# HarborC/PL-SLAM

Measured on NVIDIA H100. Metric: frames/sec (extract+match+pose-LM) 640x480, higher is better.
Workload: dtype u8/i32 front-end, f32 descriptors, f64 LM

## Files before the change

include/plslam_b200.h:

```cpp
#ifndef PLSLAM_B200_H
#define PLSLAM_B200_H
#include <stddef.h>
#include <stdint.h>
#ifdef __cplusplus
extern "C" {
#endif

#define PL_OK 0
#define PL_ERR_ARG (-1)
#define PL_ERR_CUDA (-2)
#define PL_ERR_CAPACITY (-3)

const char* pl_last_error(void);
int pl_version(void);
unsigned long long pl_launch_count(void);

typedef struct PLKeyPoint {
  float x, y, size, angle, response;
  int32_t octave, class_id;
} PLKeyPoint;

typedef struct PLOrbConfig {
  int width, height;
  int nfeatures;
  float scale_factor;
  int nlevels;
  int ini_th_fast;
  int min_th_fast;
  int max_batch;
  int cell_slot_cap;
} PLOrbConfig;

typedef struct PLOrb PLOrb;

int pl_orb_create(const PLOrbConfig* cfg, PLOrb** out);
void pl_orb_destroy(PLOrb* h);
int pl_orb_capacity(const PLOrb* h);
int pl_orb_tables(const PLOrb* h, float* scale, float* inv_scale, float* sigma2, float* inv_sigma2,
                  int* features_per_level, int* level_w, int* level_h);
int pl_orb_extract(PLOrb* h, const uint8_t* img, int stride, PLKeyPoint* kps, uint8_t* desc, int* n);
int pl_orb_extract_batch(PLOrb* h, const uint8_t* imgs, int stride, size_t frame_stride, int B,
                         PLKeyPoint* kps, uint8_t* desc, int* n);
int pl_orb_extract_batch_dev(PLOrb* h, const uint8_t* imgs, int stride, size_t frame_stride, int B,
                             PLKeyPoint* kps, uint8_t* desc, int* n, void* stream);
int pl_orb_get_level(PLOrb* h, int frame, int level, uint8_t* out, int with_border);
int pl_orb_check_overflow(PLOrb* h);
int pl_orb_debug_candidates(PLOrb* h, int frame, int level, PLKeyPoint* out, int cap);


int pl_descriptor_distance_batch(const uint8_t* a, const uint8_t* b, int n, int* out);

int pl_frame_assign_grid(const PLKeyPoint* keys_un, int n, const float* bounds, int* cell_start, int* cell_items);
int pl_frame_assign_grid_dev(const PLKeyPoint* keys_un, const int* n, int cap, int B, const float* bounds,
                             int* cell_start , int* cell_items , void* stream);

int pl_orb_search_for_initialization(const PLKeyPoint* keys1, const uint8_t* desc1, int n1, const PLKeyPoint* keys2,
                                     const uint8_t* desc2, int n2, const float* bounds, float* prev_matched,
                                     int* matches12, int window_size, float nnratio, int check_orientation);
int pl_orb_search_for_initialization_dev(const PLKeyPoint* keys1, const uint8_t* desc1, const int* n1,
                                         const PLKeyPoint* keys2, const uint8_t* desc2, const int* n2, int cap, int B,
                                         const float* bounds, float* prev_matched, int* matches12, int* nmatches,
                                         int window_size, float nnratio, int check_orientation, int* scratch,
                                         void* stream);

int pl_orb_search_by_projection_last(const PLKeyPoint* keys_cur, const uint8_t* desc_cur, int n_cur,
                                     const float* bounds, const float* Tcw, const float* K,
                                     const float* scale_factors, int nlevels, int n_last, const uint8_t* last_valid,
                                     const float* last_pos, const uint8_t* last_desc, const int* last_octave,
                                     const float* last_angle, float th, int check_orientation,
                                     const uint8_t* cur_preassigned, int* cur_match);

int pl_orb_search_by_projection_points(const PLKeyPoint* keys, const uint8_t* desc, int n, const float* bounds,
                                       const float* scale_factors, int nlevels, int n_mp, const uint8_t* in_view,
                                       const float* proj, const int* level, const float* view_cos,
                                       const uint8_t* mp_desc, float th, float nnratio, const uint8_t* preassigned,
                                       int* match);

int pl_match_bf_knn2(const uint8_t* d1, int n1, const uint8_t* d2, int n2, int* idx, int* dist);
int pl_lsd_frame_bf_match(const uint8_t* d1, int n1, const uint8_t* d2, int n2, float th, float nnratio, int* matches);
int pl_lsd_search_double(const uint8_t* d1, int n1, const uint8_t* d2, int n2, float nnratio, int* matches);
int pl_lsd_search_double_dev(const uint8_t* d1, const int* n1, const uint8_t* d2, const int* n2, int cap1, int cap2,
                             int B, float th, float nnratio, int mutual, int* matches , int* nmatches,
                             void* stream);

int pl_pose_optimization(int mode, const float* Tcw_in, const float* K, int n_points, const float* pt_obs,
                         const float* pt_inv_sigma2, const float* pt_Xw, int n_lines, const double* line_func,
                         const double* line_Xw, float* Tcw_out, uint8_t* pt_outlier, uint8_t* line_outlier,
                         int* iterations );
size_t pl_pose_optimization_scratch_doubles(int B, int cap_points, int cap_lines);
int pl_pose_optimization_dev(int mode, int B, const float* Tcw_in, const float* K, const int* n_points,
                             int cap_points, const float* pt_obs, const float* pt_inv_sigma2, const float* pt_Xw,
                             const int* n_lines, int cap_lines, const double* line_func, const double* line_Xw,
                             float* Tcw_out, uint8_t* pt_outlier, uint8_t* line_outlier, int* inliers,
                             int* iterations, double* scratch, void* stream);

typedef struct PLLineConfig {
  int width, height;
  int nfeatures;
  double min_line_length;
  int max_batch;
  int segment_cap;
  int lsd_used_in_global;
} PLLineConfig;
typedef struct PLLine PLLine;
int pl_line_create(const PLLineConfig* cfg, PLLine** out);
void pl_line_destroy(PLLine* h);
int pl_line_capacity(const PLLine* h);
int pl_line_extract(PLLine* h, const uint8_t* img, int stride, const uint8_t* mask, void* keylines, uint8_t* desc,
                    double* linefunc, int* n);
int pl_line_extract_batch(PLLine* h, const uint8_t* imgs, int stride, size_t frame_stride, int B, const uint8_t* mask,
                          void* keylines, uint8_t* desc, double* linefunc, int* n);
int pl_line_extract_batch_dev(PLLine* h, const uint8_t* imgs, int stride, size_t frame_stride, int B,
                              const uint8_t* mask, void* keylines, uint8_t* desc, double* linefunc, int* n, void* stream);
int pl_line_check_overflow(PLLine* h);
int pl_line_debug_segments(PLLine* h, int frame, float* out, int cap);
int pl_line_debug_scaled(PLLine* h, int frame, uint8_t* out, int* sw, int* sh);
int pl_line_debug_sobel(PLLine* h, int frame, short* dx, short* dy);
int pl_line_debug_order(PLLine* h, int frame, unsigned* out, int cap);
int pl_line_debug_seed_path(PLLine* h);
int pl_line_debug_fill_order(PLLine* h, int byte);

typedef struct PLFrontendConfig {
  int width, height, max_batch;
  int orb_nfeatures; float orb_scale_factor; int orb_nlevels, orb_ini_th, orb_min_th;
  int line_nfeatures; double line_min_length;
  int lm_cap_points, lm_cap_lines;
} PLFrontendConfig;
typedef struct PLFrontend PLFrontend;
int pl_frontend_create(const PLFrontendConfig* cfg, PLFrontend** out);
void pl_frontend_destroy(PLFrontend* h);
// ... 239 lines not shown
```

pl-slam_b200/binding.py:

```python
import ctypes as C
import os
import numpy as np

_HERE = os.path.dirname(os.path.abspath(__file__))
LIB_PATH = os.environ.get("PLSLAM_B200_LIB") or os.path.join(_HERE, "libplslam_b200.so")

KP_DTYPE = np.dtype([("x", "<f4"), ("y", "<f4"), ("size", "<f4"), ("angle", "<f4"),
                     ("response", "<f4"), ("octave", "<i4"), ("class_id", "<i4")])


class PLError(RuntimeError):
    pass


class PLOrbConfig(C.Structure):
    _fields_ = [("width", C.c_int), ("height", C.c_int), ("nfeatures", C.c_int), ("scale_factor", C.c_float),
                ("nlevels", C.c_int), ("ini_th_fast", C.c_int), ("min_th_fast", C.c_int), ("max_batch", C.c_int),
                ("cell_slot_cap", C.c_int)]


_lib = None
vp = C.c_void_p


def lib():
    global _lib
    if _lib is None:
        if not os.path.exists(LIB_PATH):
            raise PLError(f"{LIB_PATH} is missing: run __graft_entry__.build() (no CPU fallback exists)")
        L = C.CDLL(LIB_PATH)
        L.pl_last_error.restype = C.c_char_p
        L.pl_launch_count.restype = C.c_ulonglong
        L.pl_orb_create.argtypes = [C.POINTER(PLOrbConfig), C.POINTER(vp)]
        L.pl_orb_destroy.argtypes = [vp]
        L.pl_orb_capacity.argtypes = [vp]
        L.pl_orb_tables.argtypes = [vp] * 8
        L.pl_orb_extract.argtypes = [vp, vp, C.c_int, vp, vp, vp]
        L.pl_orb_extract_batch.argtypes = [vp, vp, C.c_int, C.c_size_t, C.c_int, vp, vp, vp]
        L.pl_orb_extract_batch_dev.argtypes = [vp, vp, C.c_int, C.c_size_t, C.c_int, vp, vp, vp, vp]
        L.pl_orb_get_level.argtypes = [vp, C.c_int, C.c_int, vp, C.c_int]
        L.pl_orb_debug_candidates.argtypes = [vp, C.c_int, C.c_int, vp, C.c_int]
        _lib = L
    return _lib


def check(rc):
    if rc < 0:
        raise PLError(f"plslam_b200 error {rc}: {lib().pl_last_error().decode()}")
    return rc


def _p(a):
    return a.ctypes.data_as(vp) if a is not None else None


def launch_count():
    return int(lib().pl_launch_count())


class ORBextractor:

    def __init__(self, nfeatures, scaleFactor, nlevels, iniThFAST, minThFAST, width=640, height=480, max_batch=1,
                 cell_slot_cap=0):
        self.cfg = PLOrbConfig(width, height, nfeatures, scaleFactor, nlevels, iniThFAST, minThFAST, max_batch,
                               cell_slot_cap)
        self._h = vp()
        check(lib().pl_orb_create(C.byref(self.cfg), C.byref(self._h)))
        self.capacity = check(lib().pl_orb_capacity(self._h))
        n = nlevels
        self._scale, self._inv, self._s2, self._is2 = (np.zeros(n, np.float32) for _ in range(4))
        self.mnFeaturesPerLevel = np.zeros(n, np.int32)
        self.level_w, self.level_h = np.zeros(n, np.int32), np.zeros(n, np.int32)
        check(lib().pl_orb_tables(self._h, _p(self._scale), _p(self._inv), _p(self._s2), _p(self._is2),
                                  _p(self.mnFeaturesPerLevel), _p(self.level_w), _p(self.level_h)))

    def __del__(self):
        if getattr(self, "_h", None) and self._h.value:
            lib().pl_orb_destroy(self._h)
            self._h = vp()

    def GetLevels(self): return self.cfg.nlevels
    def GetScaleFactor(self): return self.cfg.scale_factor
    def GetScaleFactors(self): return self._scale
    def GetInverseScaleFactors(self): return self._inv
    def GetScaleSigmaSquares(self): return self._s2
    def GetInverseScaleSigmaSquares(self): return self._is2

    def __call__(self, image, mask=None):
        image = np.ascontiguousarray(image, np.uint8)
        if image.size == 0:
            return np.zeros(0, KP_DTYPE), np.zeros((0, 32), np.uint8)
        assert image.shape == (self.cfg.height, self.cfg.width)
        kps = np.zeros(self.capacity, KP_DTYPE)
        desc = np.zeros((self.capacity, 32), np.uint8)
        n = C.c_int(0)
        check(lib().pl_orb_extract(self._h, _p(image), image.strides[0], _p(kps), _p(desc), C.byref(n)))
        return kps[:n.value].copy(), desc[:n.value].copy()

    def extract_batch(self, images):
        images = np.ascontiguousarray(images, np.uint8)
        B = images.shape[0]
        kps = np.zeros((B, self.capacity), KP_DTYPE)
        desc = np.zeros((B, self.capacity, 32), np.uint8)
        n = np.zeros(B, np.int32)
        check(lib().pl_orb_extract_batch(self._h, _p(images), images.strides[1], images.strides[0], B, _p(kps),
                                         _p(desc), _p(n)))
        return kps, desc, n

    def extract_batch_dev(self, img_ptr, stride, frame_stride, B, kps_ptr, desc_ptr, n_ptr, stream=None):
        check(lib().pl_orb_extract_batch_dev(self._h, img_ptr, stride, frame_stride, B, kps_ptr, desc_ptr, n_ptr,
                                             stream))

    def mvImagePyramid(self, level, frame=0, with_border=False):
        w, h = int(self.level_w[level]), int(self.level_h[level])
        if with_border:
            w, h = w + 38, h + 38
        out = np.zeros((h, w), np.uint8)
        check(lib().pl_orb_get_level(self._h, frame, level, _p(out), int(with_border)))
        return out

    def debug_candidates(self, level, frame=0):
        n = check(lib().pl_orb_debug_candidates(self._h, frame, level, None, 0))
        out = np.zeros(max(n, 1), KP_DTYPE)
        check(lib().pl_orb_debug_candidates(self._h, frame, level, _p(out), n))
        return out[:n]


def _u8(a):
    return np.ascontiguousarray(a, np.uint8)


def _f32(a):
    return np.ascontiguousarray(a, np.float32)


def _i32(a):
    return np.ascontiguousarray(a, np.int32)


def frame_assign_grid(keys_un, bounds):
    keys = np.ascontiguousarray(keys_un); b = _f32(bounds)
    start = np.zeros(64 * 48 + 1, np.int32); items = np.zeros(max(len(keys), 1), np.int32)
    check(lib().pl_frame_assign_grid(_p(keys), len(keys), _p(b), _p(start), _p(items)))
    return start, items[:start[-1]]


class ORBmatcher:
    TH_HIGH, TH_LOW, HISTO_LENGTH = 100, 50, 30

    def __init__(self, nnratio=0.6, checkOri=True):
        self.mfNNratio, self.mbCheckOrientation = float(nnratio), bool(checkOri)

    @staticmethod
    def DescriptorDistance(a, b):
        a, b = _u8(a).reshape(-1, 32), _u8(b).reshape(-1, 32)
        out = np.zeros(len(a), np.int32)
        check(lib().pl_descriptor_distance_batch(_p(a), _p(b), len(a), _p(out)))
        return out if len(out) > 1 else int(out[0])

    def SearchForInitialization(self, keys1, desc1, keys2, desc2, bounds, vbPrevMatched, windowSize=10):
        k1, k2 = np.ascontiguousarray(keys1), np.ascontiguousarray(keys2)
        d1, d2 = _u8(desc1), _u8(desc2)
        pm = _f32(vbPrevMatched).copy(); b = _f32(bounds)
        m = np.zeros(max(len(k1), 1), np.int32)
        f = lib().pl_orb_search_for_initialization
        f.argtypes = [vp, vp, C.c_int, vp, vp, C.c_int, vp, vp, vp, C.c_int, C.c_float, C.c_int]
        nm = check(f(_p(k1), _p(d1), len(k1), _p(k2), _p(d2), len(k2), _p(b), _p(pm), _p(m), int(windowSize),
                     self.mfNNratio, int(self.mbCheckOrientation)))
        return nm, m[:len(k1)], pm

    def SearchByProjectionLast(self, keys_cur, desc_cur, bounds, Tcw, K, scale_factors, last_valid, last_pos,
                               last_desc, last_octave, last_angle, th, preassigned=None):
        kc, dc = np.ascontiguousarray(keys_cur), _u8(desc_cur)
        arr = [_f32(bounds), _f32(Tcw), _f32(K), _f32(scale_factors), _u8(last_valid), _f32(last_pos), _u8(last_desc),
               _i32(last_octave), _f32(last_angle)]
        pre = None if preassigned is None else _u8(preassigned)
        m = np.zeros(max(len(kc), 1), np.int32)
        f = lib().pl_orb_search_by_projection_last
        f.argtypes = [vp, vp, C.c_int, vp, vp, vp, vp, C.c_int, C.c_int, vp, vp, vp, vp, vp, C.c_float, C.c_int, vp, vp]
        nm = check(f(_p(kc), _p(dc), len(kc), _p(arr[0]), _p(arr[1]), _p(arr[2]), _p(arr[3]), len(arr[3]), len(arr[4]),
                     _p(arr[4]), _p(arr[5]), _p(arr[6]), _p(arr[7]), _p(arr[8]), float(th),
                     int(self.mbCheckOrientation), _p(pre), _p(m)))
        return nm, m[:len(kc)]

    def SearchByProjectionPoints(self, keys, desc, bounds, scale_factors, in_view, proj, level, view_cos, mp_desc, th=3,
                                 preassigned=None):
        k, d = np.ascontiguousarray(keys), _u8(desc)
        arr = [_f32(bounds), _f32(scale_factors), _u8(in_view), _f32(proj), _i32(level), _f32(view_cos), _u8(mp_desc)]
        pre = None if preassigned is None else _u8(preassigned)
        m = np.zeros(max(len(k), 1), np.int32)
        f = lib().pl_orb_search_by_projection_points
        f.argtypes = [vp, vp, C.c_int, vp, vp, C.c_int, C.c_int, vp, vp, vp, vp, vp, C.c_float, C.c_float, vp, vp]
        nm = check(f(_p(k), _p(d), len(k), _p(arr[0]), _p(arr[1]), len(arr[1]), len(arr[2]), _p(arr[2]), _p(arr[3]),
                     _p(arr[4]), _p(arr[5]), _p(arr[6]), float(th), self.mfNNratio, _p(pre), _p(m)))
        return nm, m[:len(k)]


class LSDmatcher:
    TH_HIGH, TH_LOW = 80, 50

    def __init__(self, nnratio=0.7, checkOri=True):
        self.mfNNratio, self.mbCheckOrientation = float(nnratio), bool(checkOri)

    DescriptorDistance = ORBmatcher.DescriptorDistance

    @staticmethod
    def knnMatch(d1, d2):
        d1, d2 = _u8(d1), _u8(d2)
# ... 1110 lines not shown
```

pl-slam_b200/csrc/orb.cu:

```cuda

#include "common.cuh"
#include "tma.cuh"
#include "libm_glibc.cuh"
#include <math.h>
#include <vector>
#include <algorithm>
#include <string.h>

namespace pl {

constexpr int kMaxLevels = 12;
constexpr int kEdge = 19;
constexpr int kHalfPatch = 15;
constexpr int kMaxWin = 72;

__device__ char4 g_pattern[256];
__constant__ int c_umax[16];
static const int8_t h_pattern[256 * 4] = {
#include "../data/orb_pattern_31.inc"
};

struct LevelInfo {
  int w, h, pitch;
  long long off;
// ... 46 lines not shown
    int sx = tx.x, sx1 = min(sx + 1, sw - 1);
    int r0 = S0[sx] * tx.y + S0[sx1] * tx.z;
    int r1 = S1[sx] * tx.y + S1[sx1] * tx.z;
    o[k] = (uint8_t)((((b0 * (r0 >> 4)) >> 16) + ((b1 * (r1 >> 4)) >> 16) + 2) >> 2);
  }
  if (x4 + 3 < dw) {
    *reinterpret_cast<uchar4*>(D + x4) = make_uchar4(o[0], o[1], o[2], o[3]);
  } else {
    for (int k = 0; x4 + k < dw; k++) D[x4 + k] = o[k];
  }
}

__host__ __device__ __forceinline__ int fast_score_px(const uint8_t* p, int pitch, int minTh) {
  int v = p[0];
  int d0 = v - p[3 * pitch], d8 = v - p[-3 * pitch];
  if (abs(d0) <= minTh && abs(d8) <= minTh) return 0;
  int d4 = v - p[3], d12 = v - p[-3];
  if (abs(d4) <= minTh && abs(d12) <= minTh) return 0;
  int d[16];
  d[0] = d0; d[1] = v - p[3 * pitch + 1]; d[2] = v - p[2 * pitch + 2]; d[3] = v - p[pitch + 3];
  d[4] = d4; d[5] = v - p[-pitch + 3]; d[6] = v - p[-2 * pitch + 2]; d[7] = v - p[-3 * pitch + 1];
  d[8] = d8; d[9] = v - p[-3 * pitch - 1]; d[10] = v - p[-2 * pitch - 2]; d[11] = v - p[-pitch - 3];
  d[12] = d12; d[13] = v - p[pitch - 3]; d[14] = v - p[2 * pitch - 2]; d[15] = v - p[3 * pitch - 1];
  int e[16];
#pragma unroll
  for (int k = 0; k < 16; k++) e[k] = -d[k];
  int a2[16], b2[16], a4[16], b4[16];
#pragma unroll
  for (int k = 0; k < 16; k++) { a2[k] = min(d[k], d[(k + 1) & 15]); b2[k] = min(e[k], e[(k + 1) & 15]); }
#pragma unroll
  for (int k = 0; k < 16; k++) { a4[k] = min(a2[k], a2[(k + 2) & 15]); b4[k] = min(b2[k], b2[(k + 2) & 15]); }
  int bestA = -256, bestB = -256;
#pragma unroll
  for (int k = 0; k < 16; k++) {
    int a9 = min(min(a4[k], a4[(k + 4) & 15]), d[(k + 8) & 15]);
    int b9 = min(min(b4[k], b4[(k + 4) & 15]), e[(k + 8) & 15]);
    bestA = max(bestA, a9);
    bestB = max(bestB, b9);
  }
  int best = bestA > bestB ? bestA : bestB;
  int s = best - 1;
  return s >= minTh ? s : 0;
}

__device__ __forceinline__ unsigned fast_score_pair(const uint8_t* p, int pitch, int minTh) {
  auto pair = [&](int off) { return (unsigned)p[off] | ((unsigned)p[off + 1] << 16); };
  const unsigned negv = __vneg2(pair(0));
  unsigned d[16];
  d[0] = pair(3 * pitch); d[1] = pair(3 * pitch + 1); d[2] = pair(2 * pitch + 2); d[3] = pair(pitch + 3);
  d[4] = pair(3); d[5] = pair(-pitch + 3); d[6] = pair(-2 * pitch + 2); d[7] = pair(-3 * pitch + 1);
  d[8] = pair(-3 * pitch); d[9] = pair(-3 * pitch - 1); d[10] = pair(-2 * pitch - 2); d[11] = pair(-pitch - 3);
  d[12] = pair(-3); d[13] = pair(pitch - 3); d[14] = pair(2 * pitch - 2); d[15] = pair(3 * pitch - 1);
#pragma unroll
  for (int k = 0; k < 16; k++) d[k] = __vadd2(d[k], negv);
  unsigned m3[16], M3[16];
#pragma unroll
  for (int k = 0; k < 16; k++) {
    m3[k] = __vimin3_s16x2(d[k], d[(k + 1) & 15], d[(k + 2) & 15]);
    M3[k] = __vimax3_s16x2(d[k], d[(k + 1) & 15], d[(k + 2) & 15]);
  }
  unsigned best = 0x80008000u, worst = 0x7fff7fffu;
#pragma unroll
  for (int k = 0; k < 16; k += 2) {
    const unsigned a0 = __vimin3_s16x2(m3[k], m3[(k + 3) & 15], m3[(k + 6) & 15]);
    const unsigned a1 = __vimin3_s16x2(m3[k + 1], m3[(k + 4) & 15], m3[(k + 7) & 15]);
    const unsigned b0 = __vimax3_s16x2(M3[k], M3[(k + 3) & 15], M3[(k + 6) & 15]);
    const unsigned b1 = __vimax3_s16x2(M3[k + 1], M3[(k + 4) & 15], M3[(k + 7) & 15]);
    best = __vimax3_s16x2(best, a0, a1);
    worst = __vimin3_s16x2(worst, b0, b1);
  }
  unsigned out = 0;
#pragma unroll
  for (int hv = 0; hv < 2; hv++) {
    const int bb = (int)(short)(best >> (16 * hv)), ww = (int)(short)(worst >> (16 * hv));
    const int nw = 0 - ww;
    const int sc = (bb > nw ? bb : nw) - 1;
    out |= (unsigned)(sc >= minTh ? sc : 0) << (16 * hv);
  }
  return out;
}

constexpr int kFastPitchMax = 96;

__global__ void __launch_bounds__(128) k_fast_cells(OrbParams P, unsigned bulk, const CellInfo* __restrict__ cells,
                                                    const uint8_t* __restrict__ img0, int stride0, long long frame0,
                                                    const uint8_t* __restrict__ pyr, uint32_t* __restrict__ slots,
                                                    int* __restrict__ counts, int* __restrict__ overflow) {
  __shared__ __align__(128) uint8_t win_s[kMaxWin * kFastPitchMax];
  __shared__ __align__(16) uint8_t sc[kMaxWin * kFastPitchMax];
  __shared__ __align__(8) unsigned long long mbar;
  __shared__ int wsum[4];
  const int cell = blockIdx.x, frame = blockIdx.y, tid = threadIdx.x;
  CellInfo c = cells[cell];
  const LevelInfo& L = P.lv[c.level];
  const int w = c.x1 - c.x0, h = c.y1 - c.y0;
  const uint8_t* img;
  int pitch;
  if (c.level == 0) { img = img0 + (long long)frame * frame0; pitch = stride0; }
  else { img = pyr + (long long)frame * P.pyr_frame + L.off; pitch = L.pitch; }
  constexpr int WP = kFastPitchMax;
  const uint8_t* win = win_s;
  if ((bulk >> c.level) & 1u) {
    const int x0a = c.x0 & ~15, rowbytes = ((c.x1 + 15) & ~15) - x0a;
    win = win_s + (c.x0 - x0a);
    if (tid == 0) {
      tma::mbar_init(&mbar, 1);
      tma::fence_mbar_init();
      tma::mbar_expect_tx(&mbar, (unsigned)(rowbytes * h));
    }
    __syncthreads();
    if (tid < h) tma::bulk_load(win_s + tid * WP, img + (long long)(c.y0 + tid) * pitch + x0a, (unsigned)rowbytes, &mbar);
    for (int i = tid; i < (WP * h + 3) / 4; i += 128) reinterpret_cast<unsigned*>(sc)[i] = 0u;
    tma::mbar_wait(&mbar, 0);
  } else {
    const float inv_w = 1.0f / (float)w;
    for (int i = tid; i < w * h; i += 128) {
      const int y = __float2int_rz(__fmul_rn((float)i + 0.5f, inv_w)), x = i - y * w;
      win_s[y * WP + x] = img[(long long)(c.y0 + y) * pitch + c.x0 + x];
    }
    for (int i = tid; i < (WP * h + 3) / 4; i += 128) reinterpret_cast<unsigned*>(sc)[i] = 0u;
  }
  __syncthreads();
  const int dw = w - 6, dh = h - 6;
  const int npx = (dw > 0 && dh > 0) ? dw * dh : 0;
  const float inv_dw = dw > 0 ? 1.0f / (float)dw : 0.f;
  {
    const int pw = (dw + 1) >> 1, npair = (dw > 0 && dh > 0) ? pw * dh : 0;
    const float inv_pw = pw > 0 ? 1.0f / (float)pw : 0.f;
    for (int j = tid; j < npair; j += 128) {
      const int y = __float2int_rz(__fmul_rn((float)j + 0.5f, inv_pw)), x = 2 * (j - y * pw);
      const unsigned s2 = fast_score_pair(&win[(y + 3) * WP + x + 3], WP, P.minTh);
      sc[(y + 3) * WP + x + 3] = (uint8_t)(s2 & 0xffu);
      if (x + 1 < dw) sc[(y + 3) * WP + x + 4] = (uint8_t)(s2 >> 16);
    }
  }
  __syncthreads();
  int n20 = 0;
  uint8_t fl[ (kMaxWin * kMaxWin + 127) / 128 ];
  int nfl = 0;
  const int ppt = (npx + 127) / 128;
  const int beg = tid * ppt, end = min(beg + ppt, npx);
  for (int i = beg; i < end; i++) {
    int y = __float2int_rz(__fmul_rn((float)i + 0.5f, inv_dw)), x = i - y * dw;
    const uint8_t* s = &sc[(y + 3) * WP + x + 3];
    int v = s[0];
    uint8_t f = 0;
    if (v > 0 && v > s[-1] && v > s[1] && v > s[-WP - 1] && v > s[-WP] && v > s[-WP + 1] && v > s[WP - 1] &&
        v > s[WP] && v > s[WP + 1]) {
      f = (v >= P.iniTh) ? 2 : 1;
      n20 += (f == 2);
    }
    fl[nfl++] = f;
  }
  const int tot20 = __syncthreads_count(n20 > 0);
  const uint8_t need = tot20 > 0 ? 2 : 1;
  int mycount = 0;
  for (int k = 0; k < nfl; k++) mycount += (fl[k] >= need);
  int lane = tid & 31, wid = tid >> 5;
  int incl = mycount;
#pragma unroll
  for (int o = 1; o < 32; o <<= 1) { int t = __shfl_up_sync(0xffffffffu, incl, o); if (lane >= o) incl += t; }
  if (lane == 31) wsum[wid] = incl;
  __syncthreads();
  int base = 0, total = 0;
#pragma unroll
  for (int k = 0; k < 4; k++) { if (k < wid) base += wsum[k]; total += wsum[k]; }
  int pos = base + incl - mycount;
  uint32_t* out = slots + ((long long)frame * P.ncells + cell) * P.slotcap;
  for (int k = 0; k < nfl; k++) {
    if (fl[k] >= need) {
      int i = beg + k;
      int y = __float2int_rz(__fmul_rn((float)i + 0.5f, inv_dw)), x = i - y * dw;
      if (pos < P.slotcap)
        out[pos] = (uint32_t)(x + 3 + c.sx) | ((uint32_t)(y + 3 + c.sy) << 12) | ((uint32_t)sc[(y + 3) * WP + x + 3] << 24);
      pos++;
    }
  }
  if (tid == 0) {
    counts[(long long)frame * P.ncells + cell] = min(total, P.slotcap);
    if (total > P.slotcap) atomicExch(overflow, 1);
  }
}

struct QNode {
  short x0, y0, x1, y1;
  int beg, cnt;
  short prev, next;
  unsigned seq;
  unsigned char buf, noMore;
  short pad;
};
constexpr short QNIL = -1;

struct QState {
  QNode* nodes;
  short* freel;
  int nfree;
  short head, tail;
  int size;
  unsigned seq;
};

__device__ __forceinline__ short q_alloc(QState& s) { return s.freel[--s.nfree]; }
__device__ __forceinline__ void q_free(QState& s, short id, int lane) {
  if (lane == 0) s.freel[s.nfree] = id;
  s.nfree++;
}
__device__ __forceinline__ void q_push_front(QState& s, short id, int lane) {
  if (lane == 0) {
    s.nodes[id].prev = QNIL;
    s.nodes[id].next = s.head;
    if (s.head != QNIL) s.nodes[s.head].prev = id;
  }
  if (s.head == QNIL) s.tail = id;
  s.head = id;
  s.size++;
}
__device__ __forceinline__ void q_push_back(QState& s, short id, int lane) {
  if (lane == 0) {
    s.nodes[id].next = QNIL;
    s.nodes[id].prev = s.tail;
    if (s.tail != QNIL) s.nodes[s.tail].next = id;
  }
  if (s.tail == QNIL) s.head = id;
  s.tail = id;
  s.size++;
}
__device__ __forceinline__ void q_erase(QState& s, short id, int lane) {
  short p = s.nodes[id].prev, n = s.nodes[id].next;
  __syncwarp();
  if (lane == 0) {
    if (p != QNIL) s.nodes[p].next = n;
    if (n != QNIL) s.nodes[n].prev = p;
  }
  if (p == QNIL) s.head = n;
  if (n == QNIL) s.tail = p;
  s.size--;
  q_free(s, id, lane);
  __syncwarp();
}

__device__ void q_divide(QState& s, short id, uint32_t* kA, uint32_t* kB, short* vs, int& nv, int& nToExpand,
                         int lane) {
  QNode nd = s.nodes[id];
  const int halfX = (nd.x1 - nd.x0 + 1) >> 1;
  const int halfY = (nd.y1 - nd.y0 + 1) >> 1;
  const int sxp = nd.x0 + halfX, syp = nd.y0 + halfY;
  const uint32_t* src = (nd.buf ? kB : kA) + nd.beg;
  uint32_t* dst = (nd.buf ? kA : kB) + nd.beg;
  int c[4] = {0, 0, 0, 0};
  for (int i = lane; i < nd.cnt; i += 32) {
    uint32_t k = src[i];
    int kx = k & 0xfff, ky = (k >> 12) & 0xfff;
    int q = (kx < sxp) ? ((ky < syp) ? 0 : 2) : ((ky < syp) ? 1 : 3);
    c[q]++;
  }
#pragma unroll
  for (int q = 0; q < 4; q++) c[q] = warp_sum(c[q]);
  int b[4];
// ... 274 lines not shown
  if (level < 0) return;
  const LevelInfo& L = P.lv[level];
  const uint8_t* img;
  int pitch;
  if (level == 0) { img = img0 + (long long)frame * frame0; pitch = stride0; }
  else { img = pyr + (long long)frame * P.pyr_frame + L.off; pitch = L.pitch; }
  const uint32_t key = sel[((long long)frame * P.nlevels + level) * P.selcap + rank];
  const int px = (int)(key & 0xfff) + (kEdge - 3), py = (int)((key >> 12) & 0xfff) + (kEdge - 3);
  const int resp = (int)(key >> 24);
  int m10, m01 = 0;
  {
    const int u = lane - kHalfPatch;
    const uint8_t* c0 = img + (long long)py * pitch + px + u;
    int colsum = 0;
#pragma unroll
    for (int v = -kHalfPatch; v <= kHalfPatch; v++) {
      if (lane <= 2 * kHalfPatch && abs(u) <= c_umax[abs(v)]) {
        const int p = c0[v * pitch];
        colsum += p; m01 += v * p;
      }
    }
    m10 = warp_sum(u * colsum);
    m01 = warp_sum(m01);
  }
  const float angle = fast_atan2_deg((float)m01, (float)m10);
  const float factorPI = (float)(3.1415926535897932384626433832795 / 180.f);
  const float ang = __fmul_rn(angle, factorPI);
  float a = 0.f, b = 0.f;
  if (lane == 0) glibc::sincosf_(ang, &b, &a);
  a = __shfl_sync(0xffffffffu, a, 0); b = __shfl_sync(0xffffffffu, b, 0);
  const int bp = L.bpitch;
  const uint8_t* ctr = blur + (long long)frame * P.blur_frame + L.boff + (long long)py * bp + px;
  int val = 0;
#pragma unroll
  for (int k = 0; k < 8; k++) {
    const char4 pt = __ldg(&g_pattern[lane * 8 + k]);
    float x0 = (float)pt.x, y0 = (float)pt.y, x1 = (float)pt.z, y1 = (float)pt.w;
    int r0 = __float2int_rn(__fadd_rn(__fmul_rn(x0, b), __fmul_rn(y0, a)));
    int c0 = __float2int_rn(__fsub_rn(__fmul_rn(x0, a), __fmul_rn(y0, b)));
    int r1 = __float2int_rn(__fadd_rn(__fmul_rn(x1, b), __fmul_rn(y1, a)));
    int c1 = __float2int_rn(__fsub_rn(__fmul_rn(x1, a), __fmul_rn(y1, b)));
    int t0 = ctr[r0 * bp + c0], t1 = ctr[r1 * bp + c1];
    val |= (t0 < t1) << k;
  }
  desc[((long long)frame * P.cap + idx) * 32 + lane] = (uint8_t)val;
  if (lane == 0) {
    PLKeyPoint kp;
    kp.x = (float)px; kp.y = (float)py;
    if (level != 0) { kp.x = __fmul_rn(kp.x, L.scale); kp.y = __fmul_rn(kp.y, L.scale); }
    kp.size = L.size; kp.angle = angle; kp.response = (float)resp; kp.octave = level; kp.class_id = -1;
    kps[(long long)frame * P.cap + idx] = kp;
  }
}

}

using namespace pl;

struct PLOrb {
  PLOrbConfig cfg;
  OrbParams P;
  std::vector<float> scale, invScale, sigma2, invSigma2;
  std::vector<int> perLevel;
  std::vector<CellInfo> cells;
  cudaStream_t stream = nullptr;
  CellInfo* d_cells = nullptr;
  short4* d_tabs = nullptr;
  uint8_t* d_pyr = nullptr;
  uint8_t* d_blur = nullptr;
  uint32_t *d_slots = nullptr, *d_keysA = nullptr, *d_keysB = nullptr, *d_sel = nullptr;
  int *d_counts = nullptr, *d_nsel = nullptr, *d_overflow = nullptr;
  uint8_t* d_img = nullptr;
  PLKeyPoint* d_kps = nullptr;
  uint8_t* d_desc = nullptr;
  int* d_n = nullptr;
  uint8_t* h_pin = nullptr;
  size_t pin_bytes = 0;
  const uint8_t* last_img = nullptr;
  int last_stride = 0;
  long long last_frame_stride = 0;
  int last_B = 0;
  size_t quad_smem = 0;
  unsigned fast_bulk = 0;
};

static inline int cvRoundf_h(float v) { return (int)lrintf(v); }

static void build_resize_table(int s, int d, std::vector<short4>& tab) {
  double scale = (double)s / d;
  for (int i = 0; i < d; i++) {
    float f = (float)((i + 0.5) * scale - 0.5);
    int si = (int)floorf(f);
    f -= si;
    if (si < 0) { si = 0; f = 0; }
    if (si >= s - 1) { si = s - 1; f = 0; }
    short4 t;
    t.x = (short)si;
    t.y = (short)cvRoundf_h((1.f - f) * 2048);
    t.z = (short)cvRoundf_h(f * 2048);
    t.w = 0;
    tab.push_back(t);
  }
}

extern "C" int pl_orb_create(const PLOrbConfig* cfg, PLOrb** out) {
  PL_ARG(cfg && out);
  PL_ARG(cfg->width >= 64 && cfg->height >= 64 && cfg->width < 4000 && cfg->height < 4000);
  PL_ARG(cfg->nlevels >= 1 && cfg->nlevels <= kMaxLevels && cfg->nfeatures > 0 && cfg->max_batch >= 1);
  PL_ARG(cfg->scale_factor > 1.0f && cfg->min_th_fast >= 1 && cfg->ini_th_fast >= cfg->min_th_fast);
  int rc = require_device();
  if (rc) return rc;
  PLOrb* h = new PLOrb;
  h->cfg = *cfg;
  const int nl = cfg->nlevels;
  const double sf = (double)cfg->scale_factor;
  h->scale.resize(nl); h->invScale.resize(nl); h->sigma2.resize(nl); h->invSigma2.resize(nl); h->perLevel.resize(nl);
  h->scale[0] = 1.f; h->sigma2[0] = 1.f;
  for (int i = 1; i < nl; i++) { h->scale[i] = (float)(h->scale[i - 1] * sf); h->sigma2[i] = h->scale[i] * h->scale[i]; }
  for (int i = 0; i < nl; i++) { h->invScale[i] = 1.0f / h->scale[i]; h->invSigma2[i] = 1.0f / h->sigma2[i]; }
  {
    float factor = (float)(1.0f / sf);
    float nDes = cfg->nfeatures * (1 - factor) / (1 - (float)pow((double)factor, (double)nl));
    int sum = 0;
    for (int l = 0; l < nl - 1; l++) { h->perLevel[l] = cvRoundf_h(nDes); sum += h->perLevel[l]; nDes *= factor; }
    h->perLevel[nl - 1] = std::max(cfg->nfeatures - sum, 0);
  }
  int umax[16];
  {
    int v, v0, vmax = (int)floor(kHalfPatch * sqrt(2.f) / 2 + 1), vmin = (int)ceil(kHalfPatch * sqrt(2.f) / 2);
    const double hp2 = kHalfPatch * kHalfPatch;
    for (v = 0; v <= vmax; ++v) umax[v] = (int)lrint(sqrt(hp2 - v * v));
    for (v = kHalfPatch, v0 = 0; v >= vmin; --v) { while (umax[v0] == umax[v0 + 1]) ++v0; umax[v] = v0; ++v0; }
  }
  OrbParams& P = h->P;
  memset(&P, 0, sizeof(P));
  P.nlevels = nl; P.iniTh = cfg->ini_th_fast; P.minTh = cfg->min_th_fast;
  P.slotcap = cfg->cell_slot_cap > 0 ? cfg->cell_slot_cap : 128;
  P.width = cfg->width; P.height = cfg->height;
  std::vector<short4> tabs;
  long long off = 0, keyoff = 0, boff = 0;
  int maxN = 0, maxIni = 1;
  for (int l = 0; l < nl; l++) {
    LevelInfo& L = P.lv[l];
    L.w = cvRoundf_h((float)cfg->width * h->invScale[l]);
    L.h = cvRoundf_h((float)cfg->height * h->invScale[l]);
    if (L.w < 2 * kEdge + 8 || L.h < 2 * kEdge + 8) { delete h; set_error("level %d too small", l); return PL_ERR_ARG; }
    L.pitch = (L.w + 63) / 64 * 64;
    L.off = off;
    L.bpitch = L.pitch; L.boff = boff;
    boff += ((long long)L.bpitch * L.h + 255) / 256 * 256;
    if (l > 0) {
      off += (long long)L.pitch * L.h;
      off = (off + 255) / 256 * 256;
      L.tab_x = (int)tabs.size(); build_resize_table(P.lv[l - 1].w, L.w, tabs);
      L.tab_y = (int)tabs.size(); build_resize_table(P.lv[l - 1].h, L.h, tabs);
    }
    L.nfeat = h->perLevel[l];
    L.scale = h->scale[l];
    L.size = (float)(int)(31 * h->scale[l]);
    const int minBX = kEdge - 3, minBY = minBX, maxBX = L.w - kEdge + 3, maxBY = L.h - kEdge + 3;
    const float width = (float)(maxBX - minBX), height = (float)(maxBY - minBY);
    const int nCols = (int)(width / 30.f), nRows = (int)(height / 30.f);
    if (nCols < 1 || nRows < 1) { delete h; set_error("level %d has no FAST cells", l); return PL_ERR_ARG; }
    const int wCell = (int)ceilf(width / nCols), hCell = (int)ceilf(height / nRows);
    if (wCell + 6 > kMaxWin || hCell + 6 > kMaxWin) { delete h; set_error("FAST cell larger than %d", kMaxWin); return PL_ERR_ARG; }
    L.cell0 = (int)h->cells.size();
    for (int i = 0; i < nRows; i++) {
      const float iniY = (float)(minBY + i * hCell);
      float maxY = iniY + hCell + 6;
      if (iniY >= maxBY - 3) continue;
      if (maxY > maxBY) maxY = (float)maxBY;
      for (int j = 0; j < nCols; j++) {
        const float iniX = (float)(minBX + j * wCell);
        float maxX = iniX + wCell + 6;
        if (iniX >= maxBX - 6) continue;
        if (maxX > maxBX) maxX = (float)maxBX;
        CellInfo c;
        c.level = (short)l; c.x0 = (short)iniX; c.x1 = (short)maxX; c.y0 = (short)iniY; c.y1 = (short)maxY;
        c.sx = (short)(j * wCell); c.sy = (short)(i * hCell); c.pad = 0;
        h->cells.push_back(c);
      }
    }
    L.ncells = (int)h->cells.size() - L.cell0;
    L.regW = maxBX - minBX; L.regH = maxBY - minBY;
    L.nIni = (int)roundf((float)L.regW / (float)L.regH);
    if (L.nIni < 1) { delete h; set_error("aspect ratio gives 0 quadtree roots (reference divides by zero)"); return PL_ERR_ARG; }
    L.hX = (float)L.regW / L.nIni;
    L.keyoff = keyoff; L.keycap = L.ncells * P.slotcap;
    keyoff += L.keycap;
    maxN = std::max(maxN, L.nfeat); maxIni = std::max(maxIni, L.nIni);
  }
  P.ncells = (int)h->cells.size();
  P.pyr_frame = off; P.key_frame = keyoff; P.blur_frame = boff;
  auto poolcap_for = [&](int n) { return (n + 4 * maxIni + 24 + 1) & ~1; };
  auto quad_smem_for = [&](int n) {
    const int pc = poolcap_for(n);
    int p2 = 1; while (p2 < pc) p2 <<= 1;
    return (size_t)pc * sizeof(QNode) + (size_t)p2 * 8 + (size_t)pc * 6 + 64;
  };
  P.poolcap = poolcap_for(maxN);
  P.selcap = maxN + 4;
  P.cap = cfg->nfeatures + 4 * nl;
  { int p2 = 1; while (p2 < P.poolcap) p2 <<= 1; P.sortcap = p2; }
  h->quad_smem = quad_smem_for(maxN);
  {
    int dev = 0, smem_max = 0;
    cudaGetDevice(&dev);
    cudaDeviceGetAttribute(&smem_max, cudaDevAttrMaxSharedMemoryPerBlockOptin, dev);
    if (h->quad_smem > (size_t)smem_max) {
      int fit = maxN;
      while (fit > 0 && quad_smem_for(fit) > (size_t)smem_max) fit--;
      set_error("a per-level quota of %d features needs %zu B of quadtree shared memory, over the device's %d B; at most %d "
                "features fit on one level (mnFeaturesPerLevel)", maxN, h->quad_smem, smem_max, fit);
      delete h;
      return PL_ERR_ARG;
    }
  }
  const int B = cfg->max_batch;
#define ORB_TRY(e) do { int _r = (e); if (_r) { pl_orb_destroy(h); return _r; } } while (0)
#define ORB_CUDA(e) do { cudaError_t _e = (e); if (_e != cudaSuccess) { set_error("%s -> %s", #e, cudaGetErrorString(_e)); pl_orb_destroy(h); return PL_ERR_CUDA; } } while (0)
  ORB_CUDA(cudaStreamCreateWithFlags(&h->stream, cudaStreamNonBlocking));
  static_assert(sizeof(h_pattern) == sizeof(char4) * 256, "pattern size");
  ORB_CUDA(cudaMemcpyToSymbol(g_pattern, h_pattern, sizeof(h_pattern)));
  ORB_CUDA(cudaMemcpyToSymbol(c_umax, umax, sizeof(umax)));
  ORB_TRY(dev_alloc(&h->d_cells, h->cells.size()));
  ORB_CUDA(cudaMemcpy(h->d_cells, h->cells.data(), h->cells.size() * sizeof(CellInfo), cudaMemcpyHostToDevice));
  ORB_TRY(dev_alloc(&h->d_tabs, std::max<size_t>(tabs.size(), 1)));
  if (!tabs.empty()) ORB_CUDA(cudaMemcpy(h->d_tabs, tabs.data(), tabs.size() * sizeof(short4), cudaMemcpyHostToDevice));
  ORB_TRY(dev_alloc(&h->d_pyr, (size_t)std::max<long long>(off, 256) * B));
  h->fast_bulk = getenv("PLSLAM_NO_TMA") ? 0u : (((1u << nl) - 1u) & ~1u);
  ORB_TRY(dev_alloc(&h->d_blur, (size_t)boff * B));
  ORB_TRY(dev_alloc(&h->d_slots, (size_t)P.ncells * P.slotcap * B));
  ORB_TRY(dev_alloc(&h->d_counts, (size_t)P.ncells * B));
  ORB_TRY(dev_alloc(&h->d_keysA, (size_t)P.key_frame * B));
  ORB_TRY(dev_alloc(&h->d_keysB, (size_t)P.key_frame * B));
  ORB_TRY(dev_alloc(&h->d_sel, (size_t)P.selcap * nl * B));
  ORB_TRY(dev_alloc(&h->d_nsel, (size_t)nl * B));
  ORB_TRY(dev_alloc(&h->d_overflow, 1));
  ORB_CUDA(cudaMemset(h->d_overflow, 0, sizeof(int)));
  ORB_CUDA(cudaFuncSetAttribute(k_quadtree, cudaFuncAttributeMaxDynamicSharedMemorySize, (int)h->quad_smem));
  *out = h;
  return PL_OK;
}

extern "C" void pl_orb_destroy(PLOrb* h) {
  if (!h) return;
  cudaFree(h->d_cells); cudaFree(h->d_tabs); cudaFree(h->d_pyr); cudaFree(h->d_blur); cudaFree(h->d_slots); cudaFree(h->d_counts);
  cudaFree(h->d_keysA); cudaFree(h->d_keysB); cudaFree(h->d_sel); cudaFree(h->d_nsel); cudaFree(h->d_overflow);
  cudaFree(h->d_img); cudaFree(h->d_kps); cudaFree(h->d_desc); cudaFree(h->d_n);
  if (h->h_pin) cudaFreeHost(h->h_pin);
  if (h->stream) cudaStreamDestroy(h->stream);
  delete h;
}

extern "C" int pl_orb_capacity(const PLOrb* h) { return h ? h->P.cap : PL_ERR_ARG; }

extern "C" int pl_orb_tables(const PLOrb* h, float* scale, float* inv_scale, float* sigma2, float* inv_sigma2,
                             int* features_per_level, int* level_w, int* level_h) {
  PL_ARG(h);
  for (int i = 0; i < h->P.nlevels; i++) {
    if (scale) scale[i] = h->scale[i];
    if (inv_scale) inv_scale[i] = h->invScale[i];
    if (sigma2) sigma2[i] = h->sigma2[i];
    if (inv_sigma2) inv_sigma2[i] = h->invSigma2[i];
    if (features_per_level) features_per_level[i] = h->perLevel[i];
    if (level_w) level_w[i] = h->P.lv[i].w;
    if (level_h) level_h[i] = h->P.lv[i].h;
  }
  return PL_OK;
}

extern "C" int pl_orb_extract_batch_dev(PLOrb* h, const uint8_t* imgs, int stride, size_t frame_stride, int B,
                                        PLKeyPoint* kps, uint8_t* desc, int* n, void* stream_) {
  PL_ARG(h && imgs && kps && desc && n);
  PL_ARG(B >= 1 && B <= h->cfg.max_batch && stride >= h->cfg.width);
  cudaStream_t st = stream_ ? (cudaStream_t)stream_ : h->stream;
  const OrbParams& P = h->P;
  h->last_img = imgs; h->last_stride = stride; h->last_frame_stride = (long long)frame_stride; h->last_B = B;
  for (int l = 1; l < P.nlevels; l++) {
    const LevelInfo& S = P.lv[l - 1];
    const LevelInfo& D = P.lv[l];
    const uint8_t* src = (l == 1) ? imgs : h->d_pyr + S.off;
    int spitch = (l == 1) ? stride : S.pitch;
    long long sframe = (l == 1) ? (long long)frame_stride : P.pyr_frame;
    dim3 blk(64, 4), grd((D.w + 255) / 256, (D.h + 3) / 4, B);
    k_resize_level<<<grd, blk, 0, st>>>(src, spitch, sframe, S.w, S.h, h->d_pyr + D.off, D.pitch, P.pyr_frame, D.w,
                                        D.h, h->d_tabs + D.tab_x, h->d_tabs + D.tab_y);
    PL_LAUNCH_CHECK();
  }
  unsigned bulk = h->fast_bulk & ~1u;
  if (h->fast_bulk && !(((uintptr_t)imgs | (uintptr_t)stride | (uintptr_t)frame_stride) & 15)) bulk |= 1u;
  k_fast_cells<<<dim3(P.ncells, B), 128, 0, st>>>(P, bulk, h->d_cells, imgs, stride, (long long)frame_stride, h->d_pyr,
                                                  h->d_slots, h->d_counts, h->d_overflow);
  PL_LAUNCH_CHECK();
  k_quadtree<<<dim3(P.nlevels, B), 32, h->quad_smem, st>>>(P, h->d_slots, h->d_counts, h->d_keysA, h->d_keysB,
                                                           h->d_sel, h->d_nsel);
  PL_LAUNCH_CHECK();
  for (int l = 0; l < P.nlevels; l++) {
    const LevelInfo& L = P.lv[l];
    const uint8_t* src = (l == 0) ? imgs : h->d_pyr + L.off;
    k_blur_level<<<dim3((L.w + kBlurCols - 1) / kBlurCols, (L.h + kBlurTileH - 1) / kBlurTileH, B), dim3(kBlurCols, kBlurTy), 0, st>>>(
        src, (l == 0) ? stride : L.pitch, (l == 0) ? (long long)frame_stride : P.pyr_frame, L.w, L.h, h->d_blur + L.boff, L.bpitch,
        P.blur_frame);
    PL_LAUNCH_CHECK();
  }
  k_describe<<<dim3((P.cap + kDescWarps - 1) / kDescWarps, B), 32 * kDescWarps, 0, st>>>(
      P, imgs, stride, (long long)frame_stride, h->d_pyr, h->d_blur, h->d_sel, h->d_nsel, kps, desc, n);
  PL_LAUNCH_CHECK();
  return PL_OK;
}

extern "C" int pl_orb_check_overflow(PLOrb* h) {
  PL_ARG(h);
  int ov = 0;
  PL_CUDA(cudaMemcpy(&ov, h->d_overflow, sizeof(int), cudaMemcpyDeviceToHost));
  if (ov) {
    cudaMemset(h->d_overflow, 0, sizeof(int));
    set_error("a FAST cell produced more than cell_slot_cap=%d NMS maxima", h->P.slotcap);
    return PL_ERR_CAPACITY;
  }
  return PL_OK;
}

static int orb_ensure_staging(PLOrb* h) {
  if (h->d_img) return PL_OK;
  const int B = h->cfg.max_batch;
  const size_t img_bytes = (size_t)h->cfg.width * h->cfg.height;
  int rc;
  if ((rc = dev_alloc(&h->d_img, img_bytes * B))) return rc;
  if ((rc = dev_alloc(&h->d_kps, (size_t)h->P.cap * B))) return rc;
  if ((rc = dev_alloc(&h->d_desc, (size_t)h->P.cap * 32 * B))) return rc;
  if ((rc = dev_alloc(&h->d_n, (size_t)B))) return rc;
  return PL_OK;
}

extern "C" int pl_orb_extract_batch(PLOrb* h, const uint8_t* imgs, int stride, size_t frame_stride, int B,
                                    PLKeyPoint* kps, uint8_t* desc, int* n) {
  PL_ARG(h && imgs && kps && desc && n);
  PL_ARG(B >= 1 && B <= h->cfg.max_batch && stride >= h->cfg.width);
  int rc = orb_ensure_staging(h);
  if (rc) return rc;
  const int W = h->cfg.width, H = h->cfg.height;
  for (int b = 0; b < B; b++)
    PL_CUDA(cudaMemcpy2DAsync(h->d_img + (size_t)b * W * H, W, imgs + (size_t)b * frame_stride, stride, W, H,
                              cudaMemcpyHostToDevice, h->stream));
  rc = pl_orb_extract_batch_dev(h, h->d_img, W, (size_t)W * H, B, h->d_kps, h->d_desc, h->d_n, h->stream);
  if (rc) return rc;
  const size_t cap = (size_t)h->P.cap;
  PL_CUDA(cudaMemcpyAsync(kps, h->d_kps, cap * B * sizeof(PLKeyPoint), cudaMemcpyDeviceToHost, h->stream));
  PL_CUDA(cudaMemcpyAsync(desc, h->d_desc, cap * B * 32, cudaMemcpyDeviceToHost, h->stream));
  PL_CUDA(cudaMemcpyAsync(n, h->d_n, (size_t)B * sizeof(int), cudaMemcpyDeviceToHost, h->stream));
  PL_CUDA(cudaStreamSynchronize(h->stream));
  return pl_orb_check_overflow(h);
}

extern "C" int pl_orb_extract(PLOrb* h, const uint8_t* img, int stride, PLKeyPoint* kps, uint8_t* desc, int* n) {
  return pl_orb_extract_batch(h, img, stride, 0, 1, kps, desc, n);
}

extern "C" int pl_orb_get_level(PLOrb* h, int frame, int level, uint8_t* out, int with_border) {
  PL_ARG(h && out && h->last_img && frame >= 0 && frame < h->last_B && level >= 0 && level < h->P.nlevels);
  const LevelInfo& L = h->P.lv[level];
  std::vector<uint8_t> tmp((size_t)L.w * L.h);
  PL_CUDA(cudaStreamSynchronize(h->stream));
  if (level == 0)
    PL_CUDA(cudaMemcpy2D(tmp.data(), L.w, h->last_img + (size_t)frame * h->last_frame_stride, h->last_stride, L.w,
                         L.h, cudaMemcpyDeviceToHost));
  else
    PL_CUDA(cudaMemcpy2D(tmp.data(), L.w, h->d_pyr + (size_t)frame * h->P.pyr_frame + L.off, L.pitch, L.w, L.h,
                         cudaMemcpyDeviceToHost));
  if (!with_border) { memcpy(out, tmp.data(), tmp.size()); return PL_OK; }
  const int bw = L.w + 2 * kEdge, bh = L.h + 2 * kEdge;
  auto refl = [](int p, int n) { if (p < 0) p = -p; if (p >= n) p = 2 * (n - 1) - p; return p; };
  for (int y = 0; y < bh; y++)
    for (int x = 0; x < bw; x++)
      out[(size_t)y * bw + x] = tmp[(size_t)refl(y - kEdge, L.h) * L.w + refl(x - kEdge, L.w)];
  return PL_OK;
}

extern "C" int pl_orb_debug_candidates(PLOrb* h, int frame, int level, PLKeyPoint* out, int cap) {
  PL_ARG(h && frame >= 0 && frame < h->last_B && level >= 0 && level < h->P.nlevels);
  const OrbParams& P = h->P;
  const LevelInfo& L = P.lv[level];
  std::vector<int> cnt(L.ncells);
  std::vector<uint32_t> sl((size_t)L.ncells * P.slotcap);
  PL_CUDA(cudaStreamSynchronize(h->stream));
  PL_CUDA(cudaMemcpy(cnt.data(), h->d_counts + (size_t)frame * P.ncells + L.cell0, cnt.size() * sizeof(int),
                     cudaMemcpyDeviceToHost));
  PL_CUDA(cudaMemcpy(sl.data(), h->d_slots + ((size_t)frame * P.ncells + L.cell0) * P.slotcap,
                     sl.size() * sizeof(uint32_t), cudaMemcpyDeviceToHost));
  int n = 0;
  for (int c = 0; c < L.ncells; c++)
    for (int j = 0; j < cnt[c]; j++) {
      uint32_t k = sl[(size_t)c * P.slotcap + j];
      if (out && n < cap) {
        PLKeyPoint kp;
        kp.x = (float)(k & 0xfff); kp.y = (float)((k >> 12) & 0xfff); kp.size = 7.f; kp.angle = -1.f;
        kp.response = (float)(k >> 24); kp.octave = 0; kp.class_id = -1;
        out[n] = kp;
      }
      n++;
    }
  return n;
}
```

Measured before the change: 12260.

## Pack FAST NMS flags into bitmasks, zero only score borders, tune occupancy

The FAST cell kernel now keeps each thread's NMS candidate flags in two 64-bit masks instead of a per-thread local byte array, and uses popcount and find-first-set to count and emit keypoints. It also stops zeroing the whole score tile and clears only the border ring that the NMS reads. This removes local-memory spills and extra shared-memory stores. The kernel is templated on min-blocks-per-SM, picking 10 for large batches and 9 otherwise, and a debug readback for blurred levels is added.

```diff
diff --git a/include/plslam_b200.h b/include/plslam_b200.h
--- a/include/plslam_b200.h
+++ b/include/plslam_b200.h
@@ -46,6 +46,7 @@
 int pl_orb_get_level(PLOrb* h, int frame, int level, uint8_t* out, int with_border);
 int pl_orb_check_overflow(PLOrb* h);
 int pl_orb_debug_candidates(PLOrb* h, int frame, int level, PLKeyPoint* out, int cap);
+int pl_orb_debug_blurred(PLOrb* h, int frame, int level, uint8_t* out);
 
 
 int pl_descriptor_distance_batch(const uint8_t* a, const uint8_t* b, int n, int* out);
diff --git a/pl-slam_b200/binding.py b/pl-slam_b200/binding.py
--- a/pl-slam_b200/binding.py
+++ b/pl-slam_b200/binding.py
@@ -40,6 +40,7 @@
         L.pl_orb_extract_batch_dev.argtypes = [vp, vp, C.c_int, C.c_size_t, C.c_int, vp, vp, vp, vp]
         L.pl_orb_get_level.argtypes = [vp, C.c_int, C.c_int, vp, C.c_int]
         L.pl_orb_debug_candidates.argtypes = [vp, C.c_int, C.c_int, vp, C.c_int]
+        L.pl_orb_debug_blurred.argtypes = [vp, C.c_int, C.c_int, vp]
         _lib = L
     return _lib
 
@@ -124,6 +125,11 @@
         out = np.zeros(max(n, 1), KP_DTYPE)
         check(lib().pl_orb_debug_candidates(self._h, frame, level, _p(out), n))
         return out[:n]
+
+    def debug_blurred(self, level, frame=0):
+        out = np.zeros((int(self.level_h[level]), int(self.level_w[level])), np.uint8)
+        check(lib().pl_orb_debug_blurred(self._h, frame, level, _p(out)))
+        return out
 
 
 def _u8(a):
diff --git a/pl-slam_b200/csrc/orb.cu b/pl-slam_b200/csrc/orb.cu
--- a/pl-slam_b200/csrc/orb.cu
+++ b/pl-slam_b200/csrc/orb.cu
@@ -152,7 +152,8 @@
 
 constexpr int kFastPitchMax = 96;
 
-__global__ void __launch_bounds__(128) k_fast_cells(OrbParams P, unsigned bulk, const CellInfo* __restrict__ cells,
+template <int kMinBlocks>
+__global__ void __launch_bounds__(128, kMinBlocks) k_fast_cells(OrbParams P, unsigned bulk, const CellInfo* __restrict__ cells,
                                                     const uint8_t* __restrict__ img0, int stride0, long long frame0,
                                                     const uint8_t* __restrict__ pyr, uint32_t* __restrict__ slots,
                                                     int* __restrict__ counts, int* __restrict__ overflow) {
@@ -169,6 +170,12 @@
   if (c.level == 0) { img = img0 + (long long)frame * frame0; pitch = stride0; }
   else { img = pyr + (long long)frame * P.pyr_frame + L.off; pitch = L.pitch; }
   constexpr int WP = kFastPitchMax;
+  const int dw = w - 6, dh = h - 6;
+  for (int i = tid; i < 2 * (dw + 2) + 2 * dh; i += 128) {
+    if (i < dw + 2) sc[2 * WP + 2 + i] = 0;
+    else if (i < 2 * (dw + 2)) sc[(dh + 3) * WP + 2 + i - (dw + 2)] = 0;
+    else sc[(3 + ((i - 2 * (dw + 2)) >> 1)) * WP + ((i & 1) ? dw + 3 : 2)] = 0;
+  }
   const uint8_t* win = win_s;
   if ((bulk >> c.level) & 1u) {
     const int x0a = c.x0 & ~15, rowbytes = ((c.x1 + 15) & ~15) - x0a;
@@ -180,7 +187,6 @@
     }
     __syncthreads();
     if (tid < h) tma::bulk_load(win_s + tid * WP, img + (long long)(c.y0 + tid) * pitch + x0a, (unsigned)rowbytes, &mbar);
-    for (int i = tid; i < (WP * h + 3) / 4; i += 128) reinterpret_cast<unsigned*>(sc)[i] = 0u;
     tma::mbar_wait(&mbar, 0);
   } else {
     const float inv_w = 1.0f / (float)w;
@@ -188,10 +194,8 @@
       const int y = __float2int_rz(__fmul_rn((float)i + 0.5f, inv_w)), x = i - y * w;
       win_s[y * WP + x] = img[(long long)(c.y0 + y) * pitch + c.x0 + x];
     }
-    for (int i = tid; i < (WP * h + 3) / 4; i += 128) reinterpret_cast<unsigned*>(sc)[i] = 0u;
   }
   __syncthreads();
-  const int dw = w - 6, dh = h - 6;
   const int npx = (dw > 0 && dh > 0) ? dw * dh : 0;
   const float inv_dw = dw > 0 ? 1.0f / (float)dw : 0.f;
   {
@@ -205,27 +209,24 @@
     }
   }
   __syncthreads();
-  int n20 = 0;
-  uint8_t fl[ (kMaxWin * kMaxWin + 127) / 128 ];
-  int nfl = 0;
+  static_assert((kMaxWin - 6) * (kMaxWin - 6) <= 64 * 128, "NMS flags of a thread's chunk fit 64 bits");
+  unsigned long long fmin = 0, fini = 0;
   const int ppt = (npx + 127) / 128;
   const int beg = tid * ppt, end = min(beg + ppt, npx);
   for (int i = beg; i < end; i++) {
     int y = __float2int_rz(__fmul_rn((float)i + 0.5f, inv_dw)), x = i - y * dw;
     const uint8_t* s = &sc[(y + 3) * WP + x + 3];
     int v = s[0];
-    uint8_t f = 0;
     if (v > 0 && v > s[-1] && v > s[1] && v > s[-WP - 1] && v > s[-WP] && v > s[-WP + 1] && v > s[WP - 1] &&
         v > s[WP] && v > s[WP + 1]) {
-      f = (v >= P.iniTh) ? 2 : 1;
-      n20 += (f == 2);
-    }
-    fl[nfl++] = f;
-  }
-  const int tot20 = __syncthreads_count(n20 > 0);
-  const uint8_t need = tot20 > 0 ? 2 : 1;
-  int mycount = 0;
-  for (int k = 0; k < nfl; k++) mycount += (fl[k] >= need);
+      const unsigned long long bit = 1ull << (i - beg);
+      fmin |= bit;
+      if (v >= P.iniTh) fini |= bit;
+    }
+  }
+  const int tot20 = __syncthreads_count(fini != 0);
+  const unsigned long long sel = tot20 > 0 ? fini : fmin;
+  const int mycount = __popcll(sel);
   int lane = tid & 31, wid = tid >> 5;
   int incl = mycount;
 #pragma unroll
@@ -237,14 +238,11 @@
   for (int k = 0; k < 4; k++) { if (k < wid) base += wsum[k]; total += wsum[k]; }
   int pos = base + incl - mycount;
   uint32_t* out = slots + ((long long)frame * P.ncells + cell) * P.slotcap;
-  for (int k = 0; k < nfl; k++) {
-    if (fl[k] >= need) {
-      int i = beg + k;
-      int y = __float2int_rz(__fmul_rn((float)i + 0.5f, inv_dw)), x = i - y * dw;
-      if (pos < P.slotcap)
-        out[pos] = (uint32_t)(x + 3 + c.sx) | ((uint32_t)(y + 3 + c.sy) << 12) | ((uint32_t)sc[(y + 3) * WP + x + 3] << 24);
-      pos++;
-    }
+  for (unsigned long long m = sel; m; m &= m - 1, pos++) {
+    const int i = beg + __ffsll((long long)m) - 1;
+    const int y = __float2int_rz(__fmul_rn((float)i + 0.5f, inv_dw)), x = i - y * dw;
+    if (pos < P.slotcap)
+      out[pos] = (uint32_t)(x + 3 + c.sx) | ((uint32_t)(y + 3 + c.sy) << 12) | ((uint32_t)sc[(y + 3) * WP + x + 3] << 24);
   }
   if (tid == 0) {
     counts[(long long)frame * P.ncells + cell] = min(total, P.slotcap);
@@ -685,6 +683,7 @@
   int last_B = 0;
   size_t quad_smem = 0;
   unsigned fast_bulk = 0;
+  int serial_batch = 0;
 };
 
 static inline int cvRoundf_h(float v) { return (int)lrintf(v); }
@@ -810,6 +809,9 @@
     int dev = 0, smem_max = 0;
     cudaGetDevice(&dev);
     cudaDeviceGetAttribute(&smem_max, cudaDevAttrMaxSharedMemoryPerBlockOptin, dev);
+    int sms = 132;
+    cudaDeviceGetAttribute(&sms, cudaDevAttrMultiProcessorCount, dev);
+    h->serial_batch = kSerialFramesPerSM * sms;
     if (h->quad_smem > (size_t)smem_max) {
       int fit = maxN;
       while (fit > 0 && quad_smem_for(fit) > (size_t)smem_max) fit--;
@@ -893,8 +895,9 @@
   }
   unsigned bulk = h->fast_bulk & ~1u;
   if (h->fast_bulk && !(((uintptr_t)imgs | (uintptr_t)stride | (uintptr_t)frame_stride) & 15)) bulk |= 1u;
-  k_fast_cells<<<dim3(P.ncells, B), 128, 0, st>>>(P, bulk, h->d_cells, imgs, stride, (long long)frame_stride, h->d_pyr,
-                                                  h->d_slots, h->d_counts, h->d_overflow);
+  auto fast = B >= h->serial_batch ? k_fast_cells<10> : k_fast_cells<9>;
+  fast<<<dim3(P.ncells, B), 128, 0, st>>>(P, bulk, h->d_cells, imgs, stride, (long long)frame_stride, h->d_pyr, h->d_slots,
+                                          h->d_counts, h->d_overflow);
   PL_LAUNCH_CHECK();
   k_quadtree<<<dim3(P.nlevels, B), 32, h->quad_smem, st>>>(P, h->d_slots, h->d_counts, h->d_keysA, h->d_keysB,
                                                            h->d_sel, h->d_nsel);
@@ -978,6 +981,15 @@
   for (int y = 0; y < bh; y++)
     for (int x = 0; x < bw; x++)
       out[(size_t)y * bw + x] = tmp[(size_t)refl(y - kEdge, L.h) * L.w + refl(x - kEdge, L.w)];
+  return PL_OK;
+}
+
+extern "C" int pl_orb_debug_blurred(PLOrb* h, int frame, int level, uint8_t* out) {
+  PL_ARG(h && out && frame >= 0 && frame < h->last_B && level >= 0 && level < h->P.nlevels);
+  const LevelInfo& L = h->P.lv[level];
+  PL_CUDA(cudaStreamSynchronize(h->stream));
+  PL_CUDA(cudaMemcpy2D(out, L.w, h->d_blur + (size_t)frame * h->P.blur_frame + L.boff, L.bpitch, L.w, L.h,
+                       cudaMemcpyDeviceToHost));
   return PL_OK;
 }
 
```

New measurement: 12370, median of 6. No clear change (+0.8%).
